# chy980959830/Multi-Modal-Retrieval-System-Image-Search-and-Data-Governance

Hardware: AMD Instinct MI355X
Metric: images/sec encode + Mqueries/sec top-10 over 1M×512 gallery, 1→8 MI355X (higher is better)
Workload: dtype bf16; 1 GPU; ViT-B/32 bf16 encode batch 256/GPU + top-10 of 256 queries over 1000000x512 bf16 gallery rows/GPU (BASELINE configs[1]); encode_batch_per_gpu=256, gallery_rows_per_gpu=1000000, gallery_rows_total=1000000, queries=256, k=10, embed_dim=512, parallelism=single GPU, launch=single process, steps_in_flight=2, weights=seeded random init (no checkpoint reachable offline)

## Files before the change

multi-modal-retrieval-system-image-search-and-data-governance_amd/csrc/build.py:

```python
import os
import subprocess
import sys
from concurrent.futures import ThreadPoolExecutor

HERE = os.path.dirname(os.path.abspath(__file__))
SOURCES = ["api_common.cpp", "comm.cpp", "search.hip", "gemm.hip", "vit_ops.hip", "tower.hip", "preprocess.hip", "range.hip",
           "sweep.hip", "deep_topk.hip", "search_f16.hip", "range_f16.hip", "sweep_f16.hip", "decide.hip", "decide_f16.hip", "deep_qmask.hip", "sweep_qmask.hip",
           "hash_join.hip"]
LIB = os.path.join(HERE, "libmmr_hip.so")
HIPCC = os.environ.get("HIPCC", "/opt/rocm/bin/hipcc")
FLAGS = ["--offload-arch=gfx950", "-O3", "-std=c++17", "-fPIC", "-x", "hip",
         "-Wno-unused-result", "-Wno-unused-value"] + os.environ.get("MMR_EXTRA_HIPCC_FLAGS", "").split()


PER_SOURCE_FLAGS = {"vit_ops.hip": ["-mllvm", "-amdgpu-mfma-vgpr-form=1", "-fno-honor-nans"]}


def _obj(src):
    return os.path.join(HERE, "_obj", os.path.splitext(src)[0] + ".o")


def _stale(target, deps):
    if not os.path.exists(target):
        return True
    t = os.path.getmtime(target)
    return any(os.path.getmtime(d) > t for d in deps)


def build(force: bool = False, verbose: bool = True) -> str:
    os.makedirs(os.path.join(HERE, "_obj"), exist_ok=True)
    headers = [os.path.join(HERE, f) for f in os.listdir(HERE) if f.endswith((".h", ".inc"))]
    headers.append(os.path.join(HERE, "..", "..", "include", "mmr.h"))
    srcs = [s for s in SOURCES if os.path.exists(os.path.join(HERE, s))]

    def compile_one(src):
        sp, op = os.path.join(HERE, src), _obj(src)
        if force or _stale(op, [sp] + headers):
            cmd = [HIPCC] + FLAGS + PER_SOURCE_FLAGS.get(src, []) + ["-c", sp, "-o", op]
            if verbose:
                print("[mmr build]", " ".join(cmd), flush=True)
            subprocess.check_call(cmd)
            return True
        return False

    with ThreadPoolExecutor(max_workers=4) as ex:
        rebuilt = list(ex.map(compile_one, srcs))
    objs = [_obj(s) for s in srcs]
    if force or any(rebuilt) or _stale(LIB, objs):
        cmd = [HIPCC, "--offload-arch=gfx950", "-shared", "-fPIC", "-o", LIB] + objs + ["-ldl"]
        if verbose:
            print("[mmr build]", " ".join(cmd), flush=True)
        subprocess.check_call(cmd)
    return LIB


if __name__ == "__main__":
    build(force="--force" in sys.argv)
```

multi-modal-retrieval-system-image-search-and-data-governance_amd/csrc/deep_qmask.hip:

```cpp
#include "mmr_common.h"
#include "exact_dot.h"
#include "scan_pipeline.h"
#include "topk_scan_body.h"
#include "topk_scan.h"
#include "scan_host.h"

#include <hip/hip_runtime.h>

namespace mmr {

constexpr int QMASK_LDS_MAX = 160 * 1024;

template <class T, int E>
__global__ __launch_bounds__(ScanCfg<E>::THREADS, ScanCfg<E>::WAVES / 4) void scan_qm_kernel(
    const T *__restrict__ q, const T *__restrict__ gal, int Q, int64_t N, int ntiles, int tpt, int qwaves, int qpad,
    float *__restrict__ bmax, float *__restrict__ tmax, const uint32_t *__restrict__ row_masks, int64_t stride,
    const uint32_t *__restrict__ shared)
{
    scan_body<T, E, false, true>(q, gal, Q, N, ntiles, tpt, qwaves, qpad, bmax, tmax, nullptr, QMaskArgs{row_masks, stride, shared});
}

template <class T, int E>
__global__ __launch_bounds__(Scan16Cfg<E>::THREADS, 2) void scan16_qm_kernel(
    const T *__restrict__ q, const T *__restrict__ gal, int Q, int64_t N, int ntiles, int tpt, int qwaves, int qpad,
    float *__restrict__ bmax, float *__restrict__ tmax, const uint32_t *__restrict__ row_masks, int64_t stride,
    const uint32_t *__restrict__ shared)
{
    scan16_body<T, E, false, true>(q, gal, Q, N, ntiles, tpt, qwaves, qpad, bmax, tmax, nullptr, QMaskArgs{row_masks, stride, shared});
}

template <typename T, int PER>
__global__ __launch_bounds__(256) void deep_rescore_qm_kernel(const T *__restrict__ q, const T *__restrict__ gal, int64_t N,
                                                              int tile_rows, const uint32_t *__restrict__ row_mask,
                                                              const uint32_t *__restrict__ row_masks, int64_t stride,
                                                              unsigned long long *__restrict__ counter,
                                                              const uint64_t *__restrict__ tiles, int64_t tile_cap,
                                                              const double *__restrict__ thr_exact, uint64_t *__restrict__ surv_k,
                                                              uint64_t *__restrict__ surv_o, int64_t surv_cap)
{
    constexpr bool QM = true;
    const int64_t mask_stride = stride;
#include "deep_rescore_body.inc"
}

__global__ __launch_bounds__(256) void row_masks_pack_kernel(const uint8_t *__restrict__ keep, const uint32_t *__restrict__ and_mask,
                                                             int64_t N, int64_t stride, uint32_t *__restrict__ out)
{
    const int64_t qi = blockIdx.y;
    const int64_t r = (int64_t)blockIdx.x * 256 + threadIdx.x;
    const int lane = threadIdx.x & 63;
    const int64_t W = (N + 31) >> 5;
    const uint64_t bits = __ballot(r < N && keep[qi * N + (r < N ? r : 0)] != 0);
    const int64_t w = r >> 5;
    uint32_t *o = out + qi * stride;
    if ((lane & 31) == 0 && w < W) {
        uint32_t v = (uint32_t)(bits >> (lane & 32));
        if (and_mask) v &= and_mask[w];
        o[w] = v;
    }
    if (blockIdx.x == 0)
        for (int64_t p = W + threadIdx.x; p < stride; p += 256) o[p] = 0u;
}

static int ring_bytes(int E)
{
    return scan_dispatch_E(E, [&](auto e) {
        constexpr int EE = decltype(e)::value;
        if constexpr (EE == 768) return (int)Scan16Cfg<EE>::LDS;
        else return (int)ScanCfg<EE>::LDS;
    });
}

int qmask_scan_tpt(int E, int qc, int tpt)
{
    const int cap = (QMASK_LDS_MAX - ring_bytes(E)) / qmask_lds_bytes(1, qc);
    return tpt < cap ? tpt : cap;
}

template <auto K, class... A>
static int launch_qm_kernel(unsigned grid, int threads, int lds, hipStream_t st, A... args)
{
    ProfScope prof(MMR_PROF_SCAN, st);
    static DeviceOnce once;
    if (once.first()) {
        MMR_CHECK_HIP(hipFuncSetAttribute(reinterpret_cast<const void *>(K), hipFuncAttributeMaxDynamicSharedMemorySize, QMASK_LDS_MAX));
    }
    hipLaunchKernelGGL(K, dim3(grid), dim3(threads), lds, st, args...);
    MMR_CHECK_LAUNCH();
    return MMR_OK;
}

int launch_topk_scan_qmasked(mmr_dtype scan_dtype, int E, const void *q, const void *gal, int Qc, int64_t N, int ntiles, int tpt,
                             int qpad, float *bmax, float *tmax, const uint32_t *row_masks, int64_t stride,
                             const uint32_t *shared, hipStream_t st)
{
    const int lds = ring_bytes(E) + qmask_lds_bytes(tpt, qpad);
    if (scan_dtype == MMR_F32 || tpt < 1 || tpt > SCAN_MAX_TPT || lds > QMASK_LDS_MAX) {
        set_error("per-query scan: plan E=%d tpt=%d qpad=%d (%d bytes of LDS) unsupported", E, tpt, qpad, lds);
        return MMR_EIO;
    }
    const unsigned ntasks = (unsigned)((ntiles + tpt - 1) / tpt);
    return scan_dispatch_E(E, [&](auto e) {
        return dispatch_elem(scan_dtype, [&](auto tag) -> int {
            constexpr int EE = decltype(e)::value;
            using T = typename decltype(tag)::type;
            if constexpr (__is_same(T, float)) return MMR_EIO;
            else if constexpr (EE == 768)
                return launch_qm_kernel<&scan16_qm_kernel<T, EE>>(ntasks, Scan16Cfg<EE>::THREADS, lds, st, (const T *)q, (const T *)gal,
                                                                  Qc, N, ntiles, tpt, qpad / 16, qpad, bmax, tmax, row_masks, stride,
                                                                  shared);
            else
                return launch_qm_kernel<&scan_qm_kernel<T, EE>>(ntasks, ScanCfg<EE>::THREADS, lds, st, (const T *)q, (const T *)gal, Qc,
                                                                N, ntiles, tpt, qpad / 32, qpad, bmax, tmax, row_masks, stride, shared);
        });
    });
}

int launch_deep_rescore_qmasked(mmr_dtype dtype, int E, const void *q, const void *gal, int64_t N, int tile_rows,
                                const uint32_t *row_mask, const uint32_t *row_masks, int64_t stride, unsigned long long *counter,
                                const uint64_t *tiles, int64_t tile_cap, const double *thr_exact, uint64_t *surv_k,
                                uint64_t *surv_o, int64_t surv_cap, hipStream_t st)
{
    const int64_t rb = (tile_cap + 3) / 4;
    const dim3 grid((unsigned)(rb < 8192 ? rb : 8192));
    scan_dispatch_E(E, [&](auto e) {
        return dispatch_elem(dtype, [&](auto tag) -> int {
            using T = typename decltype(tag)::type;
            hipLaunchKernelGGL((deep_rescore_qm_kernel<T, decltype(e)::value / 64>), grid, dim3(256), 0, st, (const T *)q,
                               (const T *)gal, N, tile_rows, row_mask, row_masks, stride, counter, tiles, tile_cap, thr_exact, surv_k,
                               surv_o, surv_cap);
            return MMR_OK;
        });
    });
    MMR_CHECK_LAUNCH();
    return MMR_OK;
}

}

using namespace mmr;

extern "C" int mmr_row_masks_pack(const uint8_t *keep, const uint32_t *and_mask, int Q, int64_t N, int64_t stride, uint32_t *out,
                                  void *stream)
{
    const char *fn = "mmr_row_masks_pack";
    MMR_CHECK_ARG(N >= 0 && N < 0x7fffffff, "%s: N=%lld outside [0, 2^31-1)", fn, (long long)N);
    MMR_CHECK_ARG(Q >= 0 && Q <= 65535, "%s: Q=%d outside [0, 65535]", fn, Q);
    MMR_CHECK_ARG(stride >= (N + 31) / 32, "%s: stride=%lld below ceil(N/32)=%lld words", fn, (long long)stride,
                  (long long)((N + 31) / 32));
    if (Q == 0 || stride == 0) return MMR_OK;
    MMR_CHECK_ARG(out && (keep || N == 0), "%s: null pointer", fn);
    MMR_CHECK_ARG((((uintptr_t)out | (uintptr_t)and_mask) & 3) == 0, "%s: out / and_mask must be 4-byte aligned", fn);
    const int64_t bx = (N + 255) / 256;
    hipLaunchKernelGGL(row_masks_pack_kernel, dim3((unsigned)(bx > 0 ? bx : 1), (unsigned)Q), dim3(256), 0, (hipStream_t)stream, keep,
                       and_mask, N, stride, out);
    MMR_CHECK_LAUNCH();
    return MMR_OK;
}
```

multi-modal-retrieval-system-image-search-and-data-governance_amd/csrc/scan_pipeline.h:

```cpp
#pragma once
#include "mmr_common.h"

#include <type_traits>

namespace mmr {

template <int E_, int EB, int ROWS_, int WAVES_>
struct TileGeom {
    static constexpr int E = E_, ROWS = ROWS_, WAVES = WAVES_;
    static constexpr int THREADS = WAVES * 64;
    static constexpr int CH = E * EB / 16;
    static constexpr int ROWB = E * EB;
    static constexpr int TILE_BYTES = ROWS * ROWB;
    static constexpr int LOADS = ROWS * CH / 64;
    static constexpr int LPW = LOADS / WAVES;
    static_assert(LOADS % WAVES == 0, "tile loads must split evenly over the waves");
    static_assert(CH % 16 == 0, "XOR swizzle works on groups of 16 chunks");
};

__device__ __forceinline__ int swizzle(int chunk, int row) { return (chunk & ~15) | ((chunk ^ row) & 15); }

template <class G, int NIMG = 1, class T>
__device__ __forceinline__ void stage_tile(const T *src0, const T *src1, int64_t N, int tile, char *slot, int wave, int lane)
{
    constexpr int TR = G::ROWS / NIMG, EPC = 16 / sizeof(T);
    static_assert(TR % 16 == 0, "each image holds whole swizzle groups of rows");
#pragma unroll
    for (int i = 0; i < G::LPW; ++i) {
        const int instr = wave * G::LPW + i;
        const int p = instr * 64 + lane;
        const int row = p / G::CH;
        const int chunk = swizzle(p % G::CH, row);
        const int im = NIMG == 1 ? 0 : row / TR;
        int64_t grow = (int64_t)tile * TR + (row - im * TR);
        grow = grow < N ? grow : N - 1;
        glds16((im ? src1 : src0) + grow * G::E + chunk * EPC, slot + instr * 1024);
    }
}

template <int NBUF, int LPW, class Stage, class Flush, class Tile>
__device__ __forceinline__ void tile_ring(int t0, int t1, Stage &&stage, Flush &&flush, Tile &&tile)
{
    static_assert(NBUF >= 2 && NBUF <= 4, "the wait counts below assume a prefetch distance of 1 to 3 tiles");
    constexpr int PD = NBUF - 1;
#pragma unroll
    for (int i = 0; i < PD; ++i)
        if (t0 + i < t1) stage(t0 + i, i);
    int cur = 0;
    for (int t = t0; t < t1; ++t) {
        const int younger = min(PD - 1, t1 - 1 - t);
        if (younger >= 2) wait_vmcnt<2 * LPW>();
        else if (younger == 1) wait_vmcnt<LPW>();
        else wait_vmcnt<0>();
        __builtin_amdgcn_s_barrier();
        flush();
        int nxt = cur + PD; nxt = nxt >= NBUF ? nxt - NBUF : nxt;
        if (t + PD < t1) stage(t + PD, nxt);
        tile(t, cur);
        cur = cur + 1 >= NBUF ? 0 : cur + 1;
    }
}

template <int M = 15>
__device__ __forceinline__ void wait_lgkmcnt(int n, bf16x8 &a)
{
    if (n == M) asm volatile("s_waitcnt lgkmcnt(%1)" : "+v"(a) : "n"(M));
    else if constexpr (M > 0) wait_lgkmcnt<M - 1>(n, a);
}
template <int M = 15>
__device__ __forceinline__ void wait_lgkmcnt(int n, bf16x8 &a, bf16x8 &b)
{
    if (n == M) asm volatile("s_waitcnt lgkmcnt(%2)" : "+v"(a), "+v"(b) : "n"(M));
    else if constexpr (M > 0) wait_lgkmcnt<M - 1>(n, a, b);
}

__device__ __forceinline__ void ds_read_b128(bf16x8 &dst, const void *lds)
{
    asm volatile("ds_read_b128 %0, %1" : "=v"(dst) : "v"((uint32_t)(uintptr_t)lds));
}

template <class T>
__device__ __forceinline__ f32x16 mfma_32x32x16(const bf16x8 &a, const bf16x8 &b, const f32x16 &c)
{
    if constexpr (__is_same(T, f16_t))
        return __builtin_amdgcn_mfma_f32_32x32x16_f16(__builtin_bit_cast(f16x8, a), __builtin_bit_cast(f16x8, b), c, 0, 0, 0);
    else return __builtin_amdgcn_mfma_f32_32x32x16_bf16(a, b, c, 0, 0, 0);
}
template <class T>
__device__ __forceinline__ f32x4 mfma_16x16x32(const bf16x8 &a, const bf16x8 &b, const f32x4 &c)
{
    if constexpr (__is_same(T, f16_t))
        return __builtin_amdgcn_mfma_f32_16x16x32_f16(__builtin_bit_cast(f16x8, a), __builtin_bit_cast(f16x8, b), c, 0, 0, 0);
    else return __builtin_amdgcn_mfma_f32_16x16x32_bf16(a, b, c, 0, 0, 0);
}

template <int KSTEPS, int STRIDE, class T>
__device__ __forceinline__ void load_query_b16(const T *qp, bool live, bf16x8 (&bq)[KSTEPS])
{
    static_assert(sizeof(T) == 2, "16-bit elements");
#pragma unroll
    for (int s = 0; s < KSTEPS; ++s) {
        bf16x8 v = *reinterpret_cast<const bf16x8 *>(qp + s * STRIDE);
        bq[s] = live ? v : (bf16x8){0, 0, 0, 0, 0, 0, 0, 0};
    }
}

__device__ __forceinline__ void split_bf16x8(const float4 &a0, const float4 &a1, bf16x8 &hi, bf16x8 &lo)
{
    const float x[8] = {a0.x, a0.y, a0.z, a0.w, a1.x, a1.y, a1.z, a1.w};
    union { bf16x8 v; uint32_t u[4]; } h, l;
#pragma unroll
    for (int j = 0; j < 4; ++j) {
        h.u[j] = pack_bf16x2(x[2 * j], x[2 * j + 1]);
        const float r0 = x[2 * j] - __uint_as_float(h.u[j] << 16);
        const float r1 = x[2 * j + 1] - __uint_as_float(h.u[j] & 0xffff0000u);
        l.u[j] = pack_bf16x2(r0, r1);
    }
    hi = h.v;
    lo = l.v;
}

template <int KSTEPS>
__device__ __forceinline__ void load_query_split(const float *qp, bool live, bf16x8 (&bqh)[KSTEPS], bf16x8 (&bql)[KSTEPS])
{
#pragma unroll
    for (int s = 0; s < KSTEPS; ++s) {
        float4 a0 = *reinterpret_cast<const float4 *>(qp + s * 32), a1 = *reinterpret_cast<const float4 *>(qp + s * 32 + 4);
        if (!live) { a0 = make_float4(0.f, 0.f, 0.f, 0.f); a1 = a0; }
        split_bf16x8(a0, a1, bqh[s], bql[s]);
    }
}

template <int E>
using Tile32 = TileGeom<E, 2, 32, E <= 512 ? 8 : 4>;
constexpr int chains_32x32(int waves) { return waves == 4 ? 2 : 1; }

template <int E, int CHAINS, int PF, class T = bf16_t>
__device__ __forceinline__ f32x16 tile_dot_32x32(const char *trow, int c, int h, const bf16x8 (&bq)[E / 16])
{
    constexpr int KSTEPS = E / 16;
    f32x16 acc, acc2;
#pragma unroll
    for (int i = 0; i < 16; ++i) { acc[i] = 0.f; acc2[i] = 0.f; }
    bf16x8 a[PF];
    auto issue = [&](int s, bf16x8 &dst) { ds_read_b128(dst, trow + swizzle(2 * s + h, c) * 16); };
#pragma unroll
    for (int s = 0; s < PF; ++s) issue(s, a[s]);
#pragma unroll
    for (int s = 0; s < KSTEPS; ++s) {
        wait_lgkmcnt((KSTEPS - 1 - s) < (PF - 1) ? (KSTEPS - 1 - s) : (PF - 1), a[s % PF]);
        const bool second = CHAINS == 2 && (s & 1);
        if (second) acc2 = mfma_32x32x16<T>(a[s % PF], bq[s], acc2);
        else acc = mfma_32x32x16<T>(a[s % PF], bq[s], acc);
        if (s + PF < KSTEPS) {
            if (second) asm volatile("" : "+v"(acc2)); else asm volatile("" : "+v"(acc));
            issue(s + PF, a[s % PF]);
        }
    }
    if (CHAINS == 2) {
#pragma unroll
        for (int i = 0; i < 16; ++i) acc[i] += acc2[i];
    }
    return acc;
}

template <int E>
__device__ __forceinline__ f32x4 tile_dot_split3(const char *img_hi, const char *img_lo, int r, int g,
                                                 const bf16x8 (&bqh)[E / 32], const bf16x8 (&bql)[E / 32])
{
    constexpr int KSTEPS = E / 32;
    const int rowoff = r * (E * 2);
    f32x4 acc = (f32x4){0.f, 0.f, 0.f, 0.f}, acc2 = (f32x4){0.f, 0.f, 0.f, 0.f}, acc3 = (f32x4){0.f, 0.f, 0.f, 0.f};
    constexpr int PF = KSTEPS < 3 ? KSTEPS : 3;
    bf16x8 fh[PF], fl[PF];
    auto issue = [&](int s, bf16x8 &dh, bf16x8 &dl) {
        const int off = rowoff + (swizzle(4 * s + g, r) << 4);
        ds_read_b128(dh, img_hi + off);
        ds_read_b128(dl, img_lo + off);
    };
#pragma unroll
    for (int s = 0; s < PF && s < KSTEPS; ++s) issue(s, fh[s], fl[s]);
#pragma unroll
    for (int s = 0; s < KSTEPS; ++s) {
        bf16x8 &ah = fh[s % PF], &al = fl[s % PF];
        wait_lgkmcnt(2 * ((KSTEPS - 1 - s) < (PF - 1) ? (KSTEPS - 1 - s) : (PF - 1)), ah, al);
        acc = __builtin_amdgcn_mfma_f32_16x16x32_bf16(ah, bqh[s], acc, 0, 0, 0);
        acc2 = __builtin_amdgcn_mfma_f32_16x16x32_bf16(al, bqh[s], acc2, 0, 0, 0);
        acc3 = __builtin_amdgcn_mfma_f32_16x16x32_bf16(ah, bql[s], acc3, 0, 0, 0);
        if (s + PF < KSTEPS) {
            asm volatile("" : "+v"(acc), "+v"(acc2), "+v"(acc3));
            issue(s + PF, ah, al);
        }
    }
    f32x4 d;
#pragma unroll
    for (int i = 0; i < 4; ++i) d[i] = acc[i] + (acc2[i] + acc3[i]);
    return d;
}

template <bool MASKED = false>
__device__ __forceinline__ float tile_max_16(const f32x4 &acc, int t, int64_t N, int g, uint32_t bits = 0)
{
    float m = -INFINITY;
    const int64_t base = (int64_t)t * 16 + 4 * g;
#pragma unroll
    for (int i = 0; i < 4; ++i) m = fmaxf(m, base + i < N && (!MASKED || ((bits >> (4 * g + i)) & 1u)) ? acc[i] : -INFINITY);
    m = fmaxf(m, __shfl_xor(m, 16, 64));
    return fmaxf(m, __shfl_xor(m, 32, 64));
}

struct MaskWord {
    uint32_t raw;
    bool ok;
};
__device__ __forceinline__ MaskWord mask_issue(const uint32_t *row_mask, int64_t w0, int nw, int lane)
{
    const bool ok = lane < nw;
    return {row_mask[ok ? w0 + lane : 0], ok};
}
__device__ __forceinline__ uint32_t mask_take(const MaskWord &m) { return m.ok ? m.raw : 0u; }

__device__ __forceinline__ uint32_t row_mask_tile32(uint32_t words, int t, int t0, int64_t N)
{
    uint32_t w = (uint32_t)__builtin_amdgcn_readlane((int)words, t - t0);
    const int64_t left = N - (int64_t)t * 32;
    return left < 32 ? w & ((1u << (int)left) - 1u) : w;
}

__device__ __forceinline__ uint32_t row_mask_tile16(uint32_t words, int t, int t0, int64_t N)
{
    uint32_t w = (uint32_t)__builtin_amdgcn_readlane((int)words, (t >> 1) - (t0 >> 1));
    w = (w >> ((t & 1) * 16)) & 0xffffu;
// ... 59 lines not shown
```

multi-modal-retrieval-system-image-search-and-data-governance_amd/csrc/search.hip:

```cpp
#include "mmr_common.h"
#include "exact_dot.h"
#include "scan_pipeline.h"
#include "topk_scan.h"
#include "topk_scan_body.h"
#include "scan_f16.h"
#include "scan_host.h"

#include <math.h>
#include <stdlib.h>
#include <string.h>

namespace mmr {

constexpr int TILE_ROWS_F32 = 16;
constexpr int MAX_TPT = SCAN_MAX_TPT;
constexpr int KS_MAX = 32;
constexpr int K_MAX = 64;
constexpr int FIN_THREADS = 256;

__host__ __device__ static inline bool ranks_before(double sa, int64_t ia, double sb, int64_t ib) {
    return sa > sb || (sa == sb && ia < ib);
}

template <int E, bool MASKED>
__global__ __launch_bounds__(ScanCfg<E>::THREADS, ScanCfg<E>::WAVES / 4) void scan_kernel(
    const bf16_t *__restrict__ q, const bf16_t *__restrict__ gal, int Q, int64_t N, int ntiles, int tpt,
    int qwaves, int qpad, float *__restrict__ bmax, float *__restrict__ tmax, const uint32_t *__restrict__ row_mask)
{
    scan_body<bf16_t, E, MASKED>(q, gal, Q, N, ntiles, tpt, qwaves, qpad, bmax, tmax, row_mask);
}

template <int E, bool MASKED>
__global__ __launch_bounds__(Scan16Cfg<E>::THREADS, 2) void scan16_kernel(
    const bf16_t *__restrict__ q, const bf16_t *__restrict__ gal, int Q, int64_t N, int ntiles, int tpt,
    int qwaves, int qpad, float *__restrict__ bmax, float *__restrict__ tmax, const uint32_t *__restrict__ row_mask)
{
    scan16_body<bf16_t, E, MASKED>(q, gal, Q, N, ntiles, tpt, qwaves, qpad, bmax, tmax, row_mask);
}


template <int E>
struct ScanF32sCfg : TileGeom<E, 4, TILE_ROWS_F32, E <= 512 ? 8 : 4> {
    using G = TileGeom<E, 4, TILE_ROWS_F32, E <= 512 ? 8 : 4>;
    using Split = TileGeom<E, 2, 2 * TILE_ROWS_F32, G::WAVES>;
    static constexpr int IMG_BYTES = G::TILE_BYTES / 2;
    static constexpr int QMAX = G::WAVES * 16;
    static constexpr int NBUF = E <= 512 ? 3 : 2;
    static constexpr int KSTEPS = E / 32;
    static constexpr int UNITS = TILE_ROWS_F32 * (E / 16);
    static constexpr int LDS = NBUF * G::TILE_BYTES + 2 * IMG_BYTES;
    static constexpr int SPLIT_LDS = NBUF * G::TILE_BYTES;
    static_assert(Split::TILE_BYTES == G::TILE_BYTES && Split::LPW == G::LPW, "a split slot is the bytes of an fp32 tile");
};

template <int E, bool MASKED>
__global__ __launch_bounds__(ScanF32sCfg<E>::THREADS, ScanF32sCfg<E>::WAVES / 4) void scan_f32s_kernel(
    const float *__restrict__ q, const float *__restrict__ gal, int Q, int64_t N, int ntiles, int tpt, int qwaves,
    int qpad, float *__restrict__ bmax, float *__restrict__ tmax, const uint32_t *__restrict__ row_mask)
{
    using C = ScanF32sCfg<E>;
    constexpr int IMG_BYTES = C::IMG_BYTES;
    extern __shared__ __attribute__((aligned(16))) char smem[];
    char *img = smem + C::NBUF * C::TILE_BYTES;
    const int lane = threadIdx.x & 63;
    const int wave = __builtin_amdgcn_readfirstlane(threadIdx.x >> 6);
    const int r = lane & 15, g = lane >> 4;
    const int task = blockIdx.x;
    const int t0 = task * tpt;
    const int t1 = min(ntiles, t0 + tpt);
    const bool compute = wave < qwaves;

    const MaskWord mw = MASKED ? mask_issue(row_mask, t0 >> 1, ((t1 - 1) >> 1) - (t0 >> 1) + 1, lane) : MaskWord{0u, false};
    bf16x8 bqh[C::KSTEPS], bql[C::KSTEPS];
    {
        const int qrow = wave * 16 + r;
        const bool live = compute && qrow < Q;
        load_query_split<C::KSTEPS>(q + (size_t)(live ? qrow : 0) * E + g * 8, live, bqh, bql);
    }
    const uint32_t mwords = mask_take(mw);

    auto convert = [&](int slot) {
        typedef float f32x4_raw __attribute__((ext_vector_type(4)));
        const uint32_t tf = (uint32_t)(uintptr_t)(smem + slot * C::TILE_BYTES);
        const uint32_t ih = (uint32_t)(uintptr_t)img, il = ih + IMG_BYTES;
#pragma unroll
        for (int u = threadIdx.x; u < C::UNITS; u += C::THREADS) {
            const int row = u & 15, cg = u >> 4;
// ... 859 lines not shown
    int64_t rows_per_slab;
    bool fast;
    size_t off_bmax, off_tmax, off_flags, off_partial, off_seltiles, off_cand, off_meta, off_nb, off_qb, off_qres, total;
};

static bool exact_supports_E(int E) { return E == 128 || E == 256 || E == 512 || E == 768 || E == 1024; }

static SearchPlan make_plan(int64_t N, int E, int Q, int k, mmr_dtype dt)
{
    SearchPlan p{};
    p.tile_rows = dt == MMR_F32 ? TILE_ROWS_F32 : TILE_ROWS;
    p.qmax = scan_qmax(E, dt);
    p.ntiles = (int)((N + p.tile_rows - 1) / p.tile_rows);
    ScanTasks t = scan_tasks(p.ntiles);
    static const int force_tpt = getenv("MMR_SEARCH_TPT") ? atoi(getenv("MMR_SEARCH_TPT")) : 0;
    if (force_tpt >= 1 && force_tpt <= MAX_TPT) t = scan_tasks_of(p.ntiles, force_tpt);
    p.tpt = t.tpt;
    p.ntasks = t.ntasks;
    p.ks = k + 6 > KS_MAX ? KS_MAX : k + 6;
    p.fast = scan_supports_E(E) && k + 6 <= KS_MAX && N > 0;
    int nslab = (int)((N + 2047) / 2048);
    const int slab_cap = p.fast ? 16 : 64;
    p.nslab = nslab < 1 ? 1 : (nslab > slab_cap ? slab_cap : nslab);
    p.rows_per_slab = (N + p.nslab - 1) / p.nslab;
    const int qc = Q < p.qmax ? (Q + 31) / 32 * 32 : p.qmax;
    size_t off = 0;
    p.off_flags = off; off += align_up((size_t)(Q > 0 ? Q : 1) * sizeof(int32_t), 256);
    p.off_qb = off; off += align_up((size_t)(Q > 0 ? Q : 1) * E * sizeof(bf16_t), 256);
    p.off_qres = off; off += align_up((size_t)(Q > 0 ? Q : 1) * sizeof(float), 256);
    p.off_nb = off; off += 256;
    p.off_bmax = off; off += align_up((size_t)p.ntiles * qc * sizeof(float), 256);
    p.off_tmax = off; off += align_up((size_t)p.ntasks * qc * sizeof(float), 256);
    p.off_partial = off; off += align_up((size_t)(Q > 0 ? Q : 1) * p.nslab * K_MAX * sizeof(ExhEntry), 256);
    p.off_seltiles = off; off += align_up((size_t)qc * KS_MAX * sizeof(int32_t), 256);
    p.off_cand = off; off += align_up((size_t)qc * KS_MAX * TILE_ROWS * sizeof(double), 256);
    p.off_meta = off; off += align_up((size_t)qc * sizeof(FinMeta), 256);
    p.total = off;
    return p;
}

static int launch_scan_bf16(int E, const bf16_t *q, const bf16_t *gal, int Qc, int64_t N, const TopkScanGeom &g, int qpad,
                            float *bmax, float *tmax, const uint32_t *row_mask, hipStream_t st)
{
    return scan_dispatch_E(E, [&](auto e) {
        return dispatch_masked(row_mask, [&](auto m) -> int {
            constexpr int EE = decltype(e)::value;
            constexpr bool MASKED = decltype(m)::value;
            if constexpr (EE == 768)
                return launch_scan_kernel<&scan16_kernel<EE, MASKED>>(g.ntasks, Scan16Cfg<EE>::THREADS, Scan16Cfg<EE>::LDS, st, q,
                                                                      gal, Qc, N, g.ntiles, g.tpt, qpad / 16, qpad, bmax, tmax,
                                                                      row_mask);
            else
                return launch_scan_kernel<&scan_kernel<EE, MASKED>>(g.ntasks, ScanCfg<EE>::THREADS, ScanCfg<EE>::LDS, st, q, gal, Qc,
                                                                    N, g.ntiles, g.tpt, qpad / 32, qpad, bmax, tmax, row_mask);
        });
    });
}

static int launch_scan_f32(int E, const float *qf, const float *gal, const bf16_t *split_hi, const bf16_t *split_lo, int Qc,
                           int64_t N, const TopkScanGeom &g, int qpad, float *bmax, float *tmax, const int32_t *gq,
                           const uint32_t *row_mask, hipStream_t st)
{
    return scan_dispatch_E(E, [&](auto e) {
        return dispatch_masked(row_mask, [&](auto m) -> int {
            constexpr int EE = decltype(e)::value;
            constexpr bool MASKED = decltype(m)::value;
            using C = ScanF32sCfg<EE>;
            if (split_hi)
                return launch_scan_kernel<&scan_split_kernel<EE, MASKED>>(g.ntasks, C::THREADS, C::SPLIT_LDS, st, qf, split_hi,
                                                                          split_lo, Qc, N, g.ntiles, g.tpt, qpad / 16, qpad, bmax,
                                                                          tmax, gq, row_mask);
            return launch_scan_kernel<&scan_f32s_kernel<EE, MASKED>>(g.ntasks, C::THREADS, C::LDS, st, qf, gal, Qc, N, g.ntiles,
                                                                     g.tpt, qpad / 16, qpad, bmax, tmax, row_mask);
        });
    });
}

TopkScanGeom topk_scan_geom(int64_t N, int E, mmr_dtype scan_dtype) { return make_plan(N, E, 1, 1, scan_dtype); }

int launch_topk_scan(mmr_dtype scan_dtype, int E, const void *q, const void *gal, int Qc, int64_t N, const TopkScanGeom &g,
                     int qpad, float *bmax, float *tmax, const uint32_t *row_mask, hipStream_t st, const bf16_t *split_hi,
                     const bf16_t *split_lo, const int32_t *gate)
{
    if (scan_dtype == MMR_BF16) return launch_scan_bf16(E, (const bf16_t *)q, (const bf16_t *)gal, Qc, N, g, qpad, bmax, tmax, row_mask, st);
    if (scan_dtype == MMR_F16) return launch_scan_f16(E, (const f16_t *)q, (const f16_t *)gal, Qc, N, g, qpad, bmax, tmax, row_mask, st);
    return launch_scan_f32(E, (const float *)q, (const float *)gal, split_hi, split_lo, Qc, N, g, qpad, bmax, tmax, gate, row_mask, st);
}

struct TierMargin {
    const float *qres = nullptr;
    const float *gres_dev = nullptr;
    float gres_rel = 0.f;
};

template <typename T, int PER>
static int launch_finalize(const T *q, const T *gal, int Qc, int64_t N, int k, const SearchPlan &p, int qpad,
                           const float *bmax, const float *tmax, float scale, float eps_rel, const NormBound &nb, int32_t *idx,
                           float *score, double *dot64, int32_t *status, int32_t *flags, int32_t *sel_tiles,
                           double *cand, FinMeta *meta, const uint32_t *row_mask, hipStream_t st, const int32_t *gate,
                           const TierMargin &tm)
{
    ProfScope prof(MMR_PROF_FINALIZE, st);
    hipLaunchKernelGGL(select_kernel, dim3(Qc), dim3(FIN_THREADS), 0, st, p.ks, p.ntiles, p.tpt, p.ntasks, qpad, bmax,
                       tmax, sel_tiles, meta, gate);
    MMR_CHECK_LAUNCH();
    return dispatch_masked(row_mask, [&](auto m) -> int {
        constexpr bool MASKED = decltype(m)::value;
        hipLaunchKernelGGL((rescore_kernel<T, PER, MASKED>), dim3(p.ks, Qc), dim3(FIN_THREADS), 0, st, q, gal, N, p.tile_rows,
                           sel_tiles, cand, meta, gate, row_mask);
        MMR_CHECK_LAUNCH();
        hipLaunchKernelGGL(rank_kernel<MASKED>, dim3(Qc), dim3(FIN_THREADS), 0, st, N, k, p.ks, p.tile_rows, sel_tiles, cand, meta,
                           scale, eps_rel, nb.host, nb.dev, idx, score, dot64, status, flags, gate, tm.qres, tm.gres_dev,
                           tm.gres_rel, row_mask);
        MMR_CHECK_LAUNCH();
        return MMR_OK;
    });
}

template <typename T, int PER>
static int launch_exh(const T *q, const T *gal, int Q, int64_t N, int k, const SearchPlan &p, float scale,
                      const int32_t *flags, ExhEntry *partial, int32_t *idx, float *score, double *dot64,
                      const uint32_t *row_mask, hipStream_t st)
{
    ProfScope prof(MMR_PROF_EXACT, st);
    MMR_TRY(dispatch_masked(row_mask, [&](auto m) -> int {
        hipLaunchKernelGGL((exh_scan_kernel<T, PER, decltype(m)::value>), dim3(p.nslab, Q), dim3(256), 0, st, q, gal, N, k, p.nslab,
                           p.rows_per_slab, flags, partial, row_mask);
        MMR_CHECK_LAUNCH();
        return MMR_OK;
    }));
    hipLaunchKernelGGL(exh_merge_kernel, dim3(Q), dim3(FIN_THREADS), 0, st, partial, k, k, p.nslab, scale, flags, idx,
                       score, dot64);
    MMR_CHECK_LAUNCH();
    return MMR_OK;
}

int launch_norm_bound(const void *gallery, mmr_dtype dtype, int64_t N, int E, float *out, hipStream_t st)
{
    MMR_CHECK_HIP(hipMemsetAsync(out, 0, sizeof(float), st));
    if (N == 0) return MMR_OK;
    const int64_t want = (N + 3) / 4;
    const dim3 grid((unsigned)(want < 4096 ? want : 4096));
    return dispatch_elem(dtype, [&](auto tag) -> int {
        using T = typename decltype(tag)::type;
        hipLaunchKernelGGL(rownorm_max_kernel<T>, grid, dim3(256), 0, st, (const T *)gallery, N, E, (unsigned int *)out);
        MMR_CHECK_LAUNCH();
        return MMR_OK;
    });
}

struct TopkCall {
    const void *q, *gallery;
    mmr_dtype dtype;
    int Q;
    int64_t N;
    int E, k;
    float scale, eps_rel;
    NormBound nb;
    int32_t *idx;
    float *score;
    double *dot64;
    int32_t *status, *flags;
    char *ws;
    const uint32_t *row_mask;
    hipStream_t st;
};
// ... 301 lines not shown
```

multi-modal-retrieval-system-image-search-and-data-governance_amd/csrc/topk_scan_body.h:

```cpp
#pragma once
#include "mmr_common.h"
#include "scan_pipeline.h"

#include <math.h>

namespace mmr {

constexpr int TILE_ROWS = 32;
#ifndef MMR_SCAN_NBUF
#define MMR_SCAN_NBUF 3
#endif
constexpr int SCAN_NBUF = MMR_SCAN_NBUF;
#ifndef MMR_SCAN_CHAINS_FOR
#define MMR_SCAN_CHAINS_FOR(waves) chains_32x32(waves)
#endif
#ifndef MMR_SCAN_PF
#define MMR_SCAN_PF 4
#endif
static_assert(SCAN_NBUF == 3 || SCAN_NBUF == 4, "wait counts below assume a prefetch distance of 2 or 3 tiles");

constexpr int QMASK_PAD = 1;
__host__ __device__ constexpr int qmask_lds_bytes(int tpt, int qpad) { return tpt * (qpad + QMASK_PAD) * 4; }

template <int WAVES>
__device__ __forceinline__ void qmask_stage(uint32_t *__restrict__ words, const QMaskArgs &qm, int Q, int qpad, int t0, int t1,
                                            int64_t N, int wave, int lane)
{
    const int t = t0 + lane;
    const bool in = t < t1;
    uint32_t sh = 0u;
    if (in) {
        sh = qm.shared ? qm.shared[t] : 0xffffffffu;
        const int64_t left = N - (int64_t)t * TILE_ROWS;
        if (left < 32) sh &= (1u << (int)left) - 1u;
    }
    const uint32_t *src = qm.row_masks + (in ? t : t0);
    uint32_t *dst = words + lane * (qpad + QMASK_PAD);
    for (int q0 = wave * 4; q0 < qpad; q0 += WAVES * 4) {
        uint32_t w[4];
#pragma unroll
        for (int j = 0; j < 4; ++j) w[j] = q0 + j < Q ? src[(size_t)(q0 + j) * qm.stride] : 0u;
        if (in) {
#pragma unroll
            for (int j = 0; j < 4; ++j) dst[q0 + j] = w[j] & sh;
        }
    }
}
__device__ __forceinline__ void ds_read_b32(uint32_t &dst, const void *lds)
{
    asm volatile("ds_read_b32 %0, %1" : "=v"(dst) : "v"((uint32_t)(uintptr_t)lds));
}

template <int E>
struct ScanCfg : Tile32<E> {
    static_assert(E <= 512, "E = 768 runs scan16_kernel");
    static constexpr int QMAX = Tile32<E>::WAVES * 32;
    static constexpr int KSTEPS = E / 16;
    static constexpr int LDS = SCAN_NBUF * Tile32<E>::TILE_BYTES;
};

template <class T, int E, bool MASKED, bool QMASK = false>
__device__ __forceinline__ void scan_body(
    const T *__restrict__ q, const T *__restrict__ gal, int Q, int64_t N, int ntiles, int tpt,
    int qwaves, int qpad, float *__restrict__ bmax, float *__restrict__ tmax, const uint32_t *__restrict__ row_mask,
    const QMaskArgs qm = {})
{
    static_assert(!(MASKED && QMASK), "the shared mask of a per-query scan travels in QMaskArgs");
    using C = ScanCfg<E>;
    extern __shared__ __attribute__((aligned(16))) char smem[];

    const int lane = threadIdx.x & 63;
    const int wave = __builtin_amdgcn_readfirstlane(threadIdx.x >> 6);
    const int c = lane & 31, h = lane >> 5;
    const int task = blockIdx.x;
    const int t0 = task * tpt;
    const int t1 = min(ntiles, t0 + tpt);
    const bool compute = wave < qwaves;

    const MaskWord mw = MASKED ? mask_issue(row_mask, t0, t1 - t0, lane) : MaskWord{0u, false};
    bf16x8 bq[C::KSTEPS];
    {
        const int qrow = wave * 32 + c;
        const bool live = compute && qrow < Q;
        load_query_b16<C::KSTEPS, 16>(q + (size_t)(live ? qrow : 0) * E + h * 8, live, bq);
    }
    const uint32_t mwords = mask_take(mw);
    if constexpr (QMASK) {
        qmask_stage<C::WAVES>((uint32_t *)(smem + C::LDS), qm, Q, qpad, t0, t1, N, wave, lane);
        __syncthreads();
    }
    BucketMax bm{bmax, qpad, wave * 32 + c, compute, h == 0};
    tile_ring<SCAN_NBUF, C::LPW>(
        t0, t1, [&](int tile, int buf) { stage_tile<C>(gal, gal, N, tile, smem + buf * C::TILE_BYTES, wave, lane); },
        [&] { bm.flush(); },
        [&](int t, int cur) {
            if (!compute) return;
            uint32_t qw = 0u;
            if constexpr (QMASK) ds_read_b32(qw, smem + C::LDS + ((t - t0) * (qpad + QMASK_PAD) + wave * 32 + c) * 4);
            const f32x16 acc = tile_dot_32x32<E, MMR_SCAN_CHAINS_FOR(C::WAVES), MMR_SCAN_PF, T>(
                smem + cur * C::TILE_BYTES + c * C::ROWB, c, h, bq);
            float m = -INFINITY;
            if constexpr (QMASK) {
                asm volatile("s_waitcnt lgkmcnt(0)" : "+v"(qw));
                const uint32_t wh = qw >> (4 * h);
#pragma unroll
                for (int i = 0; i < 16; ++i) m = fmaxf(m, (wh >> ((i & 3) + 8 * (i >> 2))) & 1u ? acc[i] : -INFINITY);
            } else if constexpr (MASKED) {
                const uint32_t w = row_mask_tile32(mwords, t, t0, N);
                if (w == 0xffffffffu) {
#pragma unroll
                    for (int i = 0; i < 16; ++i) m = fmaxf(m, acc[i]);
                } else {
                    const uint32_t wh = w >> (4 * h);
#pragma unroll
                    for (int i = 0; i < 16; ++i) m = fmaxf(m, (wh >> ((i & 3) + 8 * (i >> 2))) & 1u ? acc[i] : -INFINITY);
                }
            } else if ((int64_t)(t + 1) * TILE_ROWS <= N) {
#pragma unroll
                for (int i = 0; i < 16; ++i) m = fmaxf(m, acc[i]);
            } else {
                const int64_t base = (int64_t)t * TILE_ROWS + 4 * h;
#pragma unroll
                for (int i = 0; i < 16; ++i) {
                    const int64_t r = base + (i & 3) + 8 * (i >> 2);
                    m = fmaxf(m, r < N ? acc[i] : -INFINITY);
                }
            }
            bm.add(t, fmaxf(m, __shfl_xor(m, 32, 64)));
        });
    bm.finish(tmax, task);
}

template <int E>
struct Scan16Cfg : TileGeom<E, 2, TILE_ROWS, 8> {
    static constexpr int QMAX = 8 * 16;
    static constexpr int KSTEPS = E / 32;
    static constexpr int LDS = SCAN_NBUF * Scan16Cfg::TILE_BYTES;
};

template <class T, int E, bool MASKED, bool QMASK = false>
__device__ __forceinline__ void scan16_body(
    const T *__restrict__ q, const T *__restrict__ gal, int Q, int64_t N, int ntiles, int tpt,
    int qwaves, int qpad, float *__restrict__ bmax, float *__restrict__ tmax, const uint32_t *__restrict__ row_mask,
    const QMaskArgs qm = {})
{
    static_assert(!(MASKED && QMASK), "the shared mask of a per-query scan travels in QMaskArgs");
    using C = Scan16Cfg<E>;
    extern __shared__ __attribute__((aligned(16))) char smem[];
    const int lane = threadIdx.x & 63;
    const int wave = __builtin_amdgcn_readfirstlane(threadIdx.x >> 6);
    const int c = lane & 15, g = lane >> 4;
    const int task = blockIdx.x;
    const int t0 = task * tpt;
    const int t1 = min(ntiles, t0 + tpt);
    const bool compute = wave < qwaves;

    const MaskWord mw = MASKED ? mask_issue(row_mask, t0, t1 - t0, lane) : MaskWord{0u, false};
    bf16x8 bq[C::KSTEPS];
    {
        const int qrow = wave * 16 + c;
        const bool live = compute && qrow < Q;
        load_query_b16<C::KSTEPS, 32>(q + (size_t)(live ? qrow : 0) * E + g * 8, live, bq);
    }
    const uint32_t mwords = mask_take(mw);
    if constexpr (QMASK) {
        qmask_stage<8>((uint32_t *)(smem + C::LDS), qm, Q, qpad, t0, t1, N, wave, lane);
        __syncthreads();
    }
    BucketMax bm{bmax, qpad, wave * 16 + c, compute, g == 0};
    tile_ring<SCAN_NBUF, C::LPW>(
        t0, t1, [&](int tile, int buf) { stage_tile<C>(gal, gal, N, tile, smem + buf * C::TILE_BYTES, wave, lane); },
        [&] { bm.flush(); },
        [&](int t, int cur) {
            if (!compute) return;
            const char *tb = smem + cur * C::TILE_BYTES;
            constexpr int NU = 2 * C::KSTEPS;
            constexpr int PF = 6;
            f32x4 acc0 = (f32x4){0.f, 0.f, 0.f, 0.f}, acc1 = (f32x4){0.f, 0.f, 0.f, 0.f};
            bf16x8 a[PF];
            uint32_t qw = 0u;
            if constexpr (QMASK) ds_read_b32(qw, smem + C::LDS + ((t - t0) * (qpad + QMASK_PAD) + wave * 16 + c) * 4);
            auto issue = [&](int u, bf16x8 &dst) {
                const int row = (u & 1) * 16 + c;
                ds_read_b128(dst, tb + row * C::ROWB + swizzle(4 * (u >> 1) + g, row) * 16);
            };
#pragma unroll
            for (int u = 0; u < PF; ++u) issue(u, a[u]);
#pragma unroll
            for (int u = 0; u < NU; ++u) {
                wait_lgkmcnt((NU - 1 - u) < (PF - 1) ? (NU - 1 - u) : (PF - 1), a[u % PF]);
                if (u & 1) acc1 = mfma_16x16x32<T>(a[u % PF], bq[u >> 1], acc1);
                else acc0 = mfma_16x16x32<T>(a[u % PF], bq[u >> 1], acc0);
                if (u + PF < NU) {
                    if (u & 1) asm volatile("" : "+v"(acc1)); else asm volatile("" : "+v"(acc0));
                    issue(u + PF, a[u % PF]);
                }
            }
            float m = -INFINITY;
            uint32_t w = 0xffffffffu;
            if constexpr (MASKED) w = row_mask_tile32(mwords, t, t0, N);
            if constexpr (QMASK) {
                asm volatile("s_waitcnt lgkmcnt(0)" : "+v"(qw));
                w = qw;
            }
            if (QMASK || (MASKED && w != 0xffffffffu)) {
                const uint32_t wg = w >> (4 * g);
#pragma unroll
                for (int i = 0; i < 4; ++i) {
                    m = fmaxf(m, (wg >> i) & 1u ? acc0[i] : -INFINITY);
                    m = fmaxf(m, (wg >> (16 + i)) & 1u ? acc1[i] : -INFINITY);
                }
            } else if (MASKED || (int64_t)(t + 1) * TILE_ROWS <= N) {
// ... 18 lines not shown
```

Measured before the change: 93390 images/s.

## Add staggered-wave tile ring to top-k scan with mid-tile barrier split

Adds a staggered variant of the gallery scan kernel in which the two halves of the waves run half a tile out of phase. A barrier is placed midway through the MFMA dot loop, so one half computes while the other stages and waits on global loads. This is meant to smooth the LDS and MFMA contention and the barrier stalls of the lockstep ring. It adds one extra ring buffer of LDS, and it is enabled by default for E<=512 when more than half the waves hold queries, with an environment variable to switch it off.

```diff
diff --git a/multi-modal-retrieval-system-image-search-and-data-governance_amd/csrc/build.py b/multi-modal-retrieval-system-image-search-and-data-governance_amd/csrc/build.py
--- a/multi-modal-retrieval-system-image-search-and-data-governance_amd/csrc/build.py
+++ b/multi-modal-retrieval-system-image-search-and-data-governance_amd/csrc/build.py
@@ -6,7 +6,7 @@
 HERE = os.path.dirname(os.path.abspath(__file__))
 SOURCES = ["api_common.cpp", "comm.cpp", "search.hip", "gemm.hip", "vit_ops.hip", "tower.hip", "preprocess.hip", "range.hip",
            "sweep.hip", "deep_topk.hip", "search_f16.hip", "range_f16.hip", "sweep_f16.hip", "decide.hip", "decide_f16.hip", "deep_qmask.hip", "sweep_qmask.hip",
-           "hash_join.hip"]
+           "hash_join.hip", "scan_stagger.hip"]
 LIB = os.path.join(HERE, "libmmr_hip.so")
 HIPCC = os.environ.get("HIPCC", "/opt/rocm/bin/hipcc")
 FLAGS = ["--offload-arch=gfx950", "-O3", "-std=c++17", "-fPIC", "-x", "hip",
diff --git a/multi-modal-retrieval-system-image-search-and-data-governance_amd/csrc/deep_qmask.hip b/multi-modal-retrieval-system-image-search-and-data-governance_amd/csrc/deep_qmask.hip
--- a/multi-modal-retrieval-system-image-search-and-data-governance_amd/csrc/deep_qmask.hip
+++ b/multi-modal-retrieval-system-image-search-and-data-governance_amd/csrc/deep_qmask.hip
@@ -3,6 +3,7 @@
 #include "scan_pipeline.h"
 #include "topk_scan_body.h"
 #include "topk_scan.h"
+#include "scan_stagger.h"
 #include "scan_host.h"
 
 #include <hip/hip_runtime.h>
@@ -100,6 +101,9 @@
         return MMR_EIO;
     }
     const unsigned ntasks = (unsigned)((ntiles + tpt - 1) / tpt);
+    if (scan_stagger_on(E, qpad / 32) && scan_stagger_ring_bytes(E) + qmask_lds_bytes(tpt, qpad) <= QMASK_LDS_MAX)
+        return launch_scan_stagger_qmasked(scan_dtype, E, q, gal, Qc, N, ntiles, tpt, ntasks, qmask_lds_bytes(tpt, qpad),
+                                           QMASK_LDS_MAX, qpad, bmax, tmax, row_masks, stride, shared, st);
     return scan_dispatch_E(E, [&](auto e) {
         return dispatch_elem(scan_dtype, [&](auto tag) -> int {
             constexpr int EE = decltype(e)::value;
diff --git a/multi-modal-retrieval-system-image-search-and-data-governance_amd/csrc/scan_pipeline.h b/multi-modal-retrieval-system-image-search-and-data-governance_amd/csrc/scan_pipeline.h
--- a/multi-modal-retrieval-system-image-search-and-data-governance_amd/csrc/scan_pipeline.h
+++ b/multi-modal-retrieval-system-image-search-and-data-governance_amd/csrc/scan_pipeline.h
@@ -61,6 +61,40 @@
     }
 }
 
+template <int NBUF, int LPW, class Stage, class Flush, class Tile>
+__device__ __forceinline__ void tile_ring_stagger(int t0, int t1, bool lag, Stage &&stage, Flush &&flush, Tile &&tile)
+{
+    static_assert(NBUF >= 3 && NBUF <= 5, "the wait counts below assume a prefetch distance of 1 to 3 tiles");
+    constexpr int PD = NBUF - 2;
+#pragma unroll
+    for (int i = 0; i < PD; ++i)
+        if (t0 + i < t1) stage(t0 + i, i);
+    auto landed = [&](int t) {
+        const int younger = min(PD - 1, t1 - 1 - t);
+        if (younger >= 2) wait_vmcnt<2 * LPW>();
+        else if (younger == 1) wait_vmcnt<LPW>();
+        else wait_vmcnt<0>();
+    };
+    if (t0 < t1) landed(t0);
+    __builtin_amdgcn_s_barrier();
+    int cur = 0;
+    for (int t = t0; t < t1; ++t) {
+        int nxt = cur + PD; nxt = nxt >= NBUF ? nxt - NBUF : nxt;
+        auto top = [&] {
+            flush();
+            if (t + PD < t1) stage(t + PD, nxt);
+        };
+        auto odd = [] { __builtin_amdgcn_s_barrier(); };
+        auto even = [&] {
+            if (t + 1 < t1) landed(t + 1);
+            __builtin_amdgcn_s_barrier();
+        };
+        if (!lag) { top(); tile(t, cur, odd); even(); }
+        else { odd(); top(); tile(t, cur, even); }
+        cur = cur + 1 >= NBUF ? 0 : cur + 1;
+    }
+}
+
 template <int M = 15>
 __device__ __forceinline__ void wait_lgkmcnt(int n, bf16x8 &a)
 {
@@ -135,8 +169,11 @@
 using Tile32 = TileGeom<E, 2, 32, E <= 512 ? 8 : 4>;
 constexpr int chains_32x32(int waves) { return waves == 4 ? 2 : 1; }
 
-template <int E, int CHAINS, int PF, class T = bf16_t>
-__device__ __forceinline__ f32x16 tile_dot_32x32(const char *trow, int c, int h, const bf16x8 (&bq)[E / 16])
+struct NoMid {
+    __device__ __forceinline__ void operator()() const {}
+};
+template <int E, int CHAINS, int PF, class T = bf16_t, class Mid = NoMid>
+__device__ __forceinline__ f32x16 tile_dot_32x32(const char *trow, int c, int h, const bf16x8 (&bq)[E / 16], Mid &&mid = Mid{})
 {
     constexpr int KSTEPS = E / 16;
     f32x16 acc, acc2;
@@ -148,6 +185,7 @@
     for (int s = 0; s < PF; ++s) issue(s, a[s]);
 #pragma unroll
     for (int s = 0; s < KSTEPS; ++s) {
+        if (s == KSTEPS / 2) mid();
         wait_lgkmcnt((KSTEPS - 1 - s) < (PF - 1) ? (KSTEPS - 1 - s) : (PF - 1), a[s % PF]);
         const bool second = CHAINS == 2 && (s & 1);
         if (second) acc2 = mfma_32x32x16<T>(a[s % PF], bq[s], acc2);
diff --git a/multi-modal-retrieval-system-image-search-and-data-governance_amd/csrc/scan_stagger.h b/multi-modal-retrieval-system-image-search-and-data-governance_amd/csrc/scan_stagger.h
--- /dev/null
+++ b/multi-modal-retrieval-system-image-search-and-data-governance_amd/csrc/scan_stagger.h
@@ -0,0 +1,15 @@
+#pragma once
+#include "mmr_common.h"
+#include "topk_scan.h"
+
+namespace mmr {
+
+bool scan_stagger_on(int E, int qwaves);
+int launch_scan_stagger(mmr_dtype scan_dtype, int E, const void *q, const void *gal, int Qc, int64_t N, const TopkScanGeom &g,
+                        int qpad, float *bmax, float *tmax, const uint32_t *row_mask, hipStream_t st);
+int scan_stagger_ring_bytes(int E);
+int launch_scan_stagger_qmasked(mmr_dtype scan_dtype, int E, const void *q, const void *gal, int Qc, int64_t N, int ntiles, int tpt,
+                                unsigned ntasks, int words_lds, int lds_max, int qpad, float *bmax, float *tmax,
+                                const uint32_t *row_masks, int64_t stride, const uint32_t *shared, hipStream_t st);
+
+}
diff --git a/multi-modal-retrieval-system-image-search-and-data-governance_amd/csrc/scan_stagger.hip b/multi-modal-retrieval-system-image-search-and-data-governance_amd/csrc/scan_stagger.hip
--- /dev/null
+++ b/multi-modal-retrieval-system-image-search-and-data-governance_amd/csrc/scan_stagger.hip
@@ -0,0 +1,93 @@
+#include "mmr_common.h"
+#include "scan_pipeline.h"
+#include "topk_scan_body.h"
+#include "topk_scan.h"
+#include "scan_stagger.h"
+#include "scan_host.h"
+
+#include <stdlib.h>
+
+namespace mmr {
+
+template <class T, int E, bool MASKED>
+__global__ __launch_bounds__(ScanCfg<E>::THREADS, ScanCfg<E>::WAVES / 4) void scan_stag_kernel(
+    const T *__restrict__ q, const T *__restrict__ gal, int Q, int64_t N, int ntiles, int tpt,
+    int qwaves, int qpad, float *__restrict__ bmax, float *__restrict__ tmax, const uint32_t *__restrict__ row_mask)
+{
+    scan_body<T, E, MASKED, false, true>(q, gal, Q, N, ntiles, tpt, qwaves, qpad, bmax, tmax, row_mask);
+}
+
+template <class T, int E>
+__global__ __launch_bounds__(ScanCfg<E>::THREADS, ScanCfg<E>::WAVES / 4) void scan_stag_qm_kernel(
+    const T *__restrict__ q, const T *__restrict__ gal, int Q, int64_t N, int ntiles, int tpt, int qwaves, int qpad,
+    float *__restrict__ bmax, float *__restrict__ tmax, const uint32_t *__restrict__ row_masks, int64_t stride,
+    const uint32_t *__restrict__ shared)
+{
+    scan_body<T, E, false, true, true>(q, gal, Q, N, ntiles, tpt, qwaves, qpad, bmax, tmax, nullptr, QMaskArgs{row_masks, stride, shared});
+}
+
+bool scan_stagger_on(int E, int qwaves)
+{
+    static const bool on = !(getenv("MMR_SCAN_STAGGER") && atoi(getenv("MMR_SCAN_STAGGER")) == 0);
+    return on && E <= 512 && qwaves > ScanCfg<128>::WAVES / 2;
+}
+
+constexpr int stag_E(int E) { return E <= 512 ? E : 512; }
+
+int scan_stagger_ring_bytes(int E)
+{
+    return scan_dispatch_E(E, [&](auto e) { return (int)ScanCfg<stag_E(decltype(e)::value)>::STAG_LDS; });
+}
+
+int launch_scan_stagger(mmr_dtype scan_dtype, int E, const void *q, const void *gal, int Qc, int64_t N, const TopkScanGeom &g,
+                        int qpad, float *bmax, float *tmax, const uint32_t *row_mask, hipStream_t st)
+{
+    MMR_CHECK_ARG(E <= 512, "staggered scan: E=%d unsupported", E);
+    return scan_dispatch_E(E, [&](auto e) {
+        return dispatch_elem(scan_dtype, [&](auto tag) -> int {
+            return dispatch_masked(row_mask, [&](auto m) -> int {
+                constexpr int EE = stag_E(decltype(e)::value);
+                constexpr bool MASKED = decltype(m)::value;
+                using T = typename decltype(tag)::type;
+                if constexpr (__is_same(T, float)) {
+                    set_error("staggered scan: E=%d dtype=%d unsupported", E, (int)scan_dtype);
+                    return MMR_EIO;
+                } else
+                    return launch_scan_kernel<&scan_stag_kernel<T, EE, MASKED>>(g.ntasks, ScanCfg<EE>::THREADS, ScanCfg<EE>::STAG_LDS, st,
+                                                                                (const T *)q, (const T *)gal, Qc, N, g.ntiles, g.tpt,
+                                                                                qpad / 32, qpad, bmax, tmax, row_mask);
+            });
+        });
+    });
+}
+
+int launch_scan_stagger_qmasked(mmr_dtype scan_dtype, int E, const void *q, const void *gal, int Qc, int64_t N, int ntiles, int tpt,
+                                unsigned ntasks, int words_lds, int lds_max, int qpad, float *bmax, float *tmax,
+                                const uint32_t *row_masks, int64_t stride, const uint32_t *shared, hipStream_t st)
+{
+    MMR_CHECK_ARG(E <= 512, "staggered per-query scan: E=%d unsupported", E);
+    return scan_dispatch_E(E, [&](auto e) {
+        return dispatch_elem(scan_dtype, [&](auto tag) -> int {
+            constexpr int EE = stag_E(decltype(e)::value);
+            using T = typename decltype(tag)::type;
+            if constexpr (__is_same(T, float)) {
+                set_error("staggered per-query scan: E=%d dtype=%d unsupported", E, (int)scan_dtype);
+                return MMR_EIO;
+            } else {
+                ProfScope prof(MMR_PROF_SCAN, st);
+                static DeviceOnce once;
+                if (once.first()) {
+                    MMR_CHECK_HIP(hipFuncSetAttribute(reinterpret_cast<const void *>(&scan_stag_qm_kernel<T, EE>),
+                                                      hipFuncAttributeMaxDynamicSharedMemorySize, lds_max));
+                }
+                hipLaunchKernelGGL((scan_stag_qm_kernel<T, EE>), dim3(ntasks), dim3(ScanCfg<EE>::THREADS),
+                                   ScanCfg<EE>::STAG_LDS + words_lds, st, (const T *)q,
+                                   (const T *)gal, Qc, N, ntiles, tpt, qpad / 32, qpad, bmax, tmax, row_masks, stride, shared);
+                MMR_CHECK_LAUNCH();
+                return MMR_OK;
+            }
+        });
+    });
+}
+
+}
diff --git a/multi-modal-retrieval-system-image-search-and-data-governance_amd/csrc/search.hip b/multi-modal-retrieval-system-image-search-and-data-governance_amd/csrc/search.hip
--- a/multi-modal-retrieval-system-image-search-and-data-governance_amd/csrc/search.hip
+++ b/multi-modal-retrieval-system-image-search-and-data-governance_amd/csrc/search.hip
@@ -3,6 +3,7 @@
 #include "scan_pipeline.h"
 #include "topk_scan.h"
 #include "topk_scan_body.h"
+#include "scan_stagger.h"
 #include "scan_f16.h"
 #include "scan_host.h"
 
@@ -1028,6 +1029,8 @@
                      int qpad, float *bmax, float *tmax, const uint32_t *row_mask, hipStream_t st, const bf16_t *split_hi,
                      const bf16_t *split_lo, const int32_t *gate)
 {
+    if (scan_dtype != MMR_F32 && scan_stagger_on(E, qpad / 32))
+        return launch_scan_stagger(scan_dtype, E, q, gal, Qc, N, g, qpad, bmax, tmax, row_mask, st);
     if (scan_dtype == MMR_BF16) return launch_scan_bf16(E, (const bf16_t *)q, (const bf16_t *)gal, Qc, N, g, qpad, bmax, tmax, row_mask, st);
     if (scan_dtype == MMR_F16) return launch_scan_f16(E, (const f16_t *)q, (const f16_t *)gal, Qc, N, g, qpad, bmax, tmax, row_mask, st);
     return launch_scan_f32(E, (const float *)q, (const float *)gal, split_hi, split_lo, Qc, N, g, qpad, bmax, tmax, gate, row_mask, st);
diff --git a/multi-modal-retrieval-system-image-search-and-data-governance_amd/csrc/topk_scan_body.h b/multi-modal-retrieval-system-image-search-and-data-governance_amd/csrc/topk_scan_body.h
--- a/multi-modal-retrieval-system-image-search-and-data-governance_amd/csrc/topk_scan_body.h
+++ b/multi-modal-retrieval-system-image-search-and-data-governance_amd/csrc/topk_scan_body.h
@@ -18,6 +18,7 @@
 #define MMR_SCAN_PF 4
 #endif
 static_assert(SCAN_NBUF == 3 || SCAN_NBUF == 4, "wait counts below assume a prefetch distance of 2 or 3 tiles");
+constexpr int SCAN_STAG_NBUF = SCAN_NBUF + 1;
 
 constexpr int QMASK_PAD = 1;
 __host__ __device__ constexpr int qmask_lds_bytes(int tpt, int qpad) { return tpt * (qpad + QMASK_PAD) * 4; }
@@ -57,9 +58,10 @@
     static constexpr int QMAX = Tile32<E>::WAVES * 32;
     static constexpr int KSTEPS = E / 16;
     static constexpr int LDS = SCAN_NBUF * Tile32<E>::TILE_BYTES;
+    static constexpr int STAG_LDS = SCAN_STAG_NBUF * Tile32<E>::TILE_BYTES;
 };
 
-template <class T, int E, bool MASKED, bool QMASK = false>
+template <class T, int E, bool MASKED, bool QMASK = false, bool STAG = false>
 __device__ __forceinline__ void scan_body(
     const T *__restrict__ q, const T *__restrict__ gal, int Q, int64_t N, int ntiles, int tpt,
     int qwaves, int qpad, float *__restrict__ bmax, float *__restrict__ tmax, const uint32_t *__restrict__ row_mask,
@@ -67,6 +69,7 @@
 {
     static_assert(!(MASKED && QMASK), "the shared mask of a per-query scan travels in QMaskArgs");
     using C = ScanCfg<E>;
+    constexpr int RING = STAG ? C::STAG_LDS : C::LDS;
     extern __shared__ __attribute__((aligned(16))) char smem[];
 
     const int lane = threadIdx.x & 63;
@@ -86,19 +89,18 @@
     }
     const uint32_t mwords = mask_take(mw);
     if constexpr (QMASK) {
-        qmask_stage<C::WAVES>((uint32_t *)(smem + C::LDS), qm, Q, qpad, t0, t1, N, wave, lane);
+        qmask_stage<C::WAVES>((uint32_t *)(smem + RING), qm, Q, qpad, t0, t1, N, wave, lane);
         __syncthreads();
     }
     BucketMax bm{bmax, qpad, wave * 32 + c, compute, h == 0};
-    tile_ring<SCAN_NBUF, C::LPW>(
-        t0, t1, [&](int tile, int buf) { stage_tile<C>(gal, gal, N, tile, smem + buf * C::TILE_BYTES, wave, lane); },
-        [&] { bm.flush(); },
-        [&](int t, int cur) {
-            if (!compute) return;
+    auto stage = [&](int tile, int buf) __attribute__((always_inline)) { stage_tile<C>(gal, gal, N, tile, smem + buf * C::TILE_BYTES, wave, lane); };
+    auto flush = [&] { bm.flush(); };
+    auto tile = [&](int t, int cur, auto &&mid) __attribute__((always_inline)) {
+            if (!compute) { mid(); return; }
             uint32_t qw = 0u;
-            if constexpr (QMASK) ds_read_b32(qw, smem + C::LDS + ((t - t0) * (qpad + QMASK_PAD) + wave * 32 + c) * 4);
+            if constexpr (QMASK) ds_read_b32(qw, smem + RING + ((t - t0) * (qpad + QMASK_PAD) + wave * 32 + c) * 4);
             const f32x16 acc = tile_dot_32x32<E, MMR_SCAN_CHAINS_FOR(C::WAVES), MMR_SCAN_PF, T>(
-                smem + cur * C::TILE_BYTES + c * C::ROWB, c, h, bq);
+                smem + cur * C::TILE_BYTES + c * C::ROWB, c, h, bq, mid);
             float m = -INFINITY;
             if constexpr (QMASK) {
                 asm volatile("s_waitcnt lgkmcnt(0)" : "+v"(qw));
@@ -118,6 +120,10 @@
             } else if ((int64_t)(t + 1) * TILE_ROWS <= N) {
 #pragma unroll
                 for (int i = 0; i < 16; ++i) m = fmaxf(m, acc[i]);
+            } else if constexpr (STAG) {
+                const uint32_t wh = ((1u << (int)(N - (int64_t)t * TILE_ROWS)) - 1u) >> (4 * h);
+#pragma unroll
+                for (int i = 0; i < 16; ++i) m = fmaxf(m, (wh >> ((i & 3) + 8 * (i >> 2))) & 1u ? acc[i] : -INFINITY);
             } else {
                 const int64_t base = (int64_t)t * TILE_ROWS + 4 * h;
 #pragma unroll
@@ -127,7 +133,9 @@
                 }
             }
             bm.add(t, fmaxf(m, __shfl_xor(m, 32, 64)));
-        });
+        };
+    if constexpr (STAG) tile_ring_stagger<SCAN_STAG_NBUF, C::LPW>(t0, t1, wave >= C::WAVES / 2, stage, flush, tile);
+    else tile_ring<SCAN_NBUF, C::LPW>(t0, t1, stage, flush, [&](int t, int cur) { tile(t, cur, NoMid{}); });
     bm.finish(tmax, task);
 }
 
```

Result: no change. 92900 images/s (-0.5%).
